# Veason-silverbullet/DIGAT

Hardware: AMD Instinct MI355X
Metric: MIND dev impressions scored/sec (AUC match not run) (higher is better)
Workload: dtype f32; 1 GPU; MIND-small default: --graph_encoder=DIGAT neighbors=3 hops=2 (N=10, U=67), d=400, graph_depth=3, fp32 dev inference; projection=auto -> fp16x3, N=10, U=67, d=400, graph_depth=3, news_num=65238, parallelism=dp1 (row shards, no data-path collective), ranks_in_process_group=1

## Files before the change

digat_amd/_lib.py:

```python
from __future__ import annotations

import ctypes as C
import os
from typing import Optional

import torch

_HERE = os.path.dirname(os.path.abspath(__file__))
LIB_PATH = os.environ.get("DIGAT_HIP_LIB") or os.path.join(_HERE, "lib", "libdigat_hip.so")
DIGAT_MAX_DEPTH = 16
DIGAT_MAX_NODES = 128
GEMM_BF16X6, GEMM_F16X3 = 0, 1
GEMM_F16F8C = 2
PARAMS_GEMM_F16X3 = 64
PARAMS_BD_TILED = 128
PARAMS_PQ_FP8 = 256
PARAMS_SIDE_STREAM_OFF, PARAMS_SIDE_STREAM_ON = 512, 1024
PARAMS_NO_LIVE_ROWS = 2048
PARAMS_PROJ_F16F8C = 4096

_f = C.c_void_p


class LayerParams(C.Structure):
    _fields_ = [(k, _f) for k in ("W", "bW", "F1", "F2", "F3", "b3", "a", "wsplit", "f3_wsplit")]


class MsaParams(C.Structure):
    _fields_ = ([(k, C.c_int32) for k in ("word_embedding_dim", "head_num", "head_dim", "attention_dim")]
                + [(k, C.c_void_p) for k in ("word_embedding", "W_Q", "b_Q", "W_K", "W_V", "b_V", "A1", "b1", "a2",
                                             "qkv_wsplit", "a1_wsplit")])


class CnnParams(C.Structure):
    _fields_ = ([(k, C.c_int32) for k in ("word_embedding_dim", "kernel_num", "taps", "attention_dim")]
                + [(k, C.c_void_p) for k in ("word_embedding", "W", "b", "A1", "b1", "a2", "w_split", "a1_wsplit")])


class SplitJob(C.Structure):
    _fields_ = [("w0", C.c_void_p), ("w1", C.c_void_p), ("w2", C.c_void_p), ("rows", C.c_int32), ("cols", C.c_int32), ("layout", C.c_int32),
                ("reserved", C.c_int32), ("image", C.c_void_p)]


class GatherJob(C.Structure):
    _fields_ = [("src", C.c_void_p), ("dst", C.c_void_p), ("row_bytes", C.c_int64), ("rows", C.c_int64),
                ("idx", C.c_void_p), ("idx2", C.c_void_p), ("inner", C.c_int64)]


class Params(C.Structure):
    _fields_ = ([("d", C.c_int32), ("depth", C.c_int32), ("category_num", C.c_int32), ("flags", C.c_int32)]
                + [(k, _f) for k in ("topic_node_embedding", "cand_K", "cand_Q", "cand_bQ",
                                     "news_graph_W", "news_graph_b", "user_news_K", "user_news_Q",
# ... 107 lines not shown
    "digat_xattn_pairwise_bwd_workspace": (C.c_size_t, [C.c_int] * 3),
    "digat_xattn_pairwise_bwd": (C.c_int, [_f] * 11 + [C.c_float] + [_f] * 4 + [C.c_int] * 4 + [_f, C.c_size_t, _f]),
    "digat_sum_nodes": (C.c_int, [_f, _f, C.c_int, C.c_int, C.c_int, _f]),
    "digat_xattn_train_save_bytes": (C.c_size_t, [C.c_int] * 3),
    "digat_xattn_train_workspace_bytes": (C.c_size_t, [C.c_int] * 3),
    "digat_xattn_fwd_train": (C.c_int, [_f] * 11 + [C.c_float, C.c_uint32, C.c_float, C.c_uint32] + [C.c_int] * 3 + [_f, C.c_size_t, _f, C.c_size_t, _f, C.c_int,
                                        _f]),
    "digat_xattn_bwd": (C.c_int, [_f] * 10 + [C.c_float, C.c_float, _f, C.c_size_t] + [_f] * 9 + [C.c_int] * 3 + [_f, C.c_size_t, _f, C.c_int, _f]),
    "digat_opt_chunk": (C.c_int, []),
    "digat_clip_adam_step": (C.c_int, [_f, _f, _f, C.c_int, _f] + [C.c_float] * 5 + [C.c_int, _f]),
    "digat_row_logits_bwd": (C.c_int, [_f] * 5 + [C.c_int, C.c_int, _f]),
    "digat_click_loss": (C.c_int, [_f, C.c_int, C.c_int, _f, _f, _f]),
    "digat_split_job_bytes": (C.c_size_t, [C.c_int] * 4),
    "digat_split_jobs": (C.c_int, [C.POINTER(SplitJob), C.c_int, _f]),
    "digat_news_ctx_train_save_bytes": (C.c_size_t, [C.c_int] * 3),
    "digat_news_ctx_train_workspace_bytes": (C.c_size_t, [C.c_int] * 3),
    "digat_news_ctx_fwd_train": (C.c_int, [_f] * 8 + [C.c_float, C.c_uint32] + [C.c_int] * 3 + [_f, C.c_size_t, _f, C.c_size_t, _f, _f]),
    "digat_news_ctx_bwd": (C.c_int, [_f] * 6 + [C.c_float, _f, C.c_size_t] + [_f] * 6 + [C.c_int] * 4 + [_f, C.c_size_t, _f]),
    "digat_user_ctx_train_save_bytes": (C.c_size_t, [C.c_int] * 5),
    "digat_user_ctx_train_workspace_bytes": (C.c_size_t, [C.c_int] * 5),
    "digat_user_ctx_fwd_train": (C.c_int, [_f] * 13 + [C.c_float, C.c_uint32] + [C.c_int] * 5 + [_f, C.c_size_t, _f, C.c_size_t, _f, _f, _f]),
    "digat_user_ctx_bwd": (C.c_int, [_f] * 10 + [C.c_float, _f, C.c_size_t] + [_f] * 10 + [C.c_int] * 6 + [_f, C.c_size_t, _f, _f]),
    "digat_profile_start": (C.c_int, [C.c_int]),
    "digat_profile_stop": (C.c_int, [C.POINTER(C.c_double), C.POINTER(C.c_double), C.POINTER(C.c_int)]),
    "digat_profile_set_kinds": (C.c_int, [C.c_uint]),
    "digat_profile_gemm_bytes": (C.c_int, [C.POINTER(C.c_double)]),
    "digat_profile_marker": (C.c_int, [C.c_int, _f]),
    "digat_encoder_shared_workspace_bytes": (C.c_size_t, [C.c_int] * 6),
    "digat_encoder_fwd_shared": (C.c_int, [C.POINTER(Params)] + [_f] * 10 + [C.c_int] * 3 + [_f, C.c_size_t, _f]),
    "digat_user_row_runs": (C.c_int, [_f] * 4 + [C.c_int] * 5 + [_f] * 4 + [C.c_size_t, _f]),
    "digat_profile_xattn_parts": (C.c_int, [C.POINTER(C.c_double), C.POINTER(C.c_double), C.POINTER(C.c_int)]),
    "digat_split_ctx_fused_bytes": (C.c_size_t, [C.c_int]),
    "digat_split_ctx_fused_weights": (C.c_int, [_f, C.c_int, _f, _f]),
}
KERNEL_KINDS = ("proj", "linear", "xattn", "pool", "topic", "glue", "agg")
XATTN_PARTS = ("twin", "l0", "news", "other")
EXPORTED = tuple(_SIGNATURES)
ABI_VERSION = 4


def lib() -> C.CDLL:
    global _lib
    if _lib is None:
        if not os.path.exists(LIB_PATH):
            raise DigatHipError(
                f"{LIB_PATH} is missing: the HIP extension has not been built "
                "(run `python -m digat_amd.build` or __graft_entry__.build()). There is no CPU fallback.")
        handle = C.CDLL(LIB_PATH)
        handle.digat_version.restype, handle.digat_version.argtypes = C.c_int, []
        got = handle.digat_version()
        if got != ABI_VERSION:
            raise DigatHipError(f"{LIB_PATH} reports ABI version {got}, this loader's signature table is for version {ABI_VERSION}: "
                                "rebuild it from this tree (python -m digat_amd.build)")
        for name, (res, args) in _SIGNATURES.items():
            fn = getattr(handle, name)
            fn.restype, fn.argtypes = res, args
        _lib = handle
    return _lib


EXT_PATH = os.path.join(_HERE, "lib", "digat_torch_ext.so")
USE_TORCH_EXT = os.environ.get("DIGAT_TORCH_EXT", "1") != "0"
_ext = None


def ext():
# ... 97 lines not shown
```

digat_amd/csrc/digat_kernels.hip:

```cpp
#include <hip/hip_runtime.h>
#include <stdint.h>
#include <string.h>
#include <stdlib.h>
#include <atomic>
#include <initializer_list>
#include <mutex>
#include <unordered_map>
#include <utility>

#include "../../include/digat_hip.h"

typedef float v4f __attribute__((ext_vector_type(4)));

#define DIGAT_CHECK_LAUNCH()                                   \
    do {                                                       \
        if (hipGetLastError() != hipSuccess) return DIGAT_ERR_LAUNCH; \
    } while (0)

static inline size_t align_up(size_t v, size_t a) { return (v + a - 1) / a * a; }
struct Arena {
    char* base; size_t cap, used; bool ok;
    Arena() : base(nullptr), cap(SIZE_MAX), used(0), ok(true) {}
    Arena(void* p, size_t n) : base((char*)p), cap(n), used(0), ok(p != nullptr) {}
    template <class T> T* take(size_t count) {
// ... 102 lines not shown
}
__device__ __forceinline__ void wait_vmcnt(int n) {
    switch (n) {
        case 0: asm volatile("s_waitcnt vmcnt(0)" ::: "memory"); break;
        case 1: asm volatile("s_waitcnt vmcnt(1)" ::: "memory"); break;
        case 2: asm volatile("s_waitcnt vmcnt(2)" ::: "memory"); break;
        case 3: asm volatile("s_waitcnt vmcnt(3)" ::: "memory"); break;
        case 4: asm volatile("s_waitcnt vmcnt(4)" ::: "memory"); break;
        case 5: asm volatile("s_waitcnt vmcnt(5)" ::: "memory"); break;
        case 6: asm volatile("s_waitcnt vmcnt(6)" ::: "memory"); break;
        default: asm volatile("s_waitcnt vmcnt(4)" ::: "memory"); break;
    }
}

#ifndef DIGAT_TWIN_R
#define DIGAT_TWIN_R 2
#endif
__device__ __forceinline__ float leaky02_uniform(float e) {
    const float t = 0.2f * e;
    float r;
    asm("v_max_f32 %0, %1, %2" : "=v"(r) : "s"(e), "v"(t));
    return r;
}
__device__ __forceinline__ unsigned hash32(unsigned x) {
    x ^= x >> 16; x *= 0x7feb352dU; x ^= x >> 15; x *= 0x846ca68bU; x ^= x >> 16;
    return x;
}
__host__ __device__ __forceinline__ unsigned drop_threshold(float p) { return (unsigned)(p * 4294967296.0); }
__device__ __forceinline__ bool drop_keep(unsigned seed, long e, unsigned thr) {
    return hash32((unsigned)e * 0x9E3779B9U + hash32(seed + (unsigned)(e >> 32))) >= thr;
}
constexpr int TWIN_R = DIGAT_TWIN_R;
#include "digat_gemm.inc"
#include "digat_xattn.inc"
#include "digat_context.inc"
#include "digat_ctxfused.inc"
#include "digat_glue.inc"

extern "C" {

int digat_version(void) { return DIGAT_ABI_VERSION; }

const char* digat_error_string(int code) {
    switch (code) {
        case DIGAT_OK: return "ok";
        case DIGAT_ERR_ARG: return "bad argument (null pointer or negative size)";
        case DIGAT_ERR_SHAPE: return "unsupported shape (d % 4 != 0, graph larger than DIGAT_MAX_NODES, depth too large)";
        case DIGAT_ERR_WORKSPACE: return "workspace too small";
        case DIGAT_ERR_LAUNCH: return "HIP kernel launch failed";
        default: return "unknown error";
    }
}

int digat_linear_f32(const float* x, int64_t ldx, const float* w, const float* b, float* y, int64_t ldy,
                     int M, int N, int K, void* stream) {
    if (!x || !w || !y || M < 0 || N <= 0 || K <= 0) return DIGAT_ERR_ARG;
    if (K % 4 || ldx % 4) return DIGAT_ERR_SHAPE;
    return launch_gemm(gemm_plain(x, ldx, w, b, y, ldy, M, N, K, 0), (hipStream_t)stream);
}

struct XattnWs { float *h, *P, *Q, *r, *alpha; };
static XattnWs xattn_carve(Arena& a, int B, int n, int d) {
    const size_t nd = (size_t)B * n * d;
    XattnWs w{};
    w.h = a.take<float>(3 * nd);
    if (w.h) { w.P = w.h + nd; w.Q = w.P + nd; }
    w.r = a.take<float>((size_t)B * d);
    w.alpha = a.take<float>((size_t)B * n * n);
    return w;
}
size_t digat_xattn_workspace_bytes(int B, int n, int d) { Arena a; xattn_carve(a, B, n, d); return a.used; }

int digat_xattn_pairwise_fwd(const float* Pr, const float* Q, const float* h, const float* X,
                             const float* a, const uint8_t* A, float* out, float* alpha,
                             int B, int n, int d, void* stream) {
    if (!Pr || !Q || !h || !X || !a || !A || !out || !alpha) return DIGAT_ERR_ARG;
    return launch_xattn_pairwise(Pr, Q, h, X, a, A, out, alpha, B, n, d, (hipStream_t)stream);
}

struct TwinLists { const unsigned* word; const int* list; const int* count; };

struct XattnOpts {
    const void* wsplit = nullptr;
    const int* rowidx = nullptr; const int* nrows_dev = nullptr; const uint8_t* live = nullptr;
    int sparse_mode = DIGAT_XATTN_DENSE; const int* sparse_flag = nullptr;
    int pq_x3 = 0, pq_mode = 0, centre_limit = 0, gemm_format = 0, prof_part = 0;
    unsigned* range_flag = nullptr; const TwinLists* tw = nullptr;
};

static int xattn_core(const float* X, const uint8_t* A, const float* r_given,
                      const float* W, const float* bW, const float* F1, const float* F2, const float* a,
// ... 485 lines not shown
    const bool xu0_grouped = Xg0 != nullptr;
    const int d = p->d, C = p->category_num, L = p->depth, U = H + C, C1 = C + 1;
    const int fmt = (p->flags & DIGAT_PARAMS_GEMM_F16X3) ? 1 : 0;
    unsigned* const rflag = fmt ? (unsigned*)p->range_flag : nullptr;
    const int lfmt = (p->flags & DIGAT_PARAMS_PROJ_F16F8C) ? DIGAT_GEMM_F16F8C : fmt;
    const int bd_disp = (p->flags & DIGAT_PARAMS_BD_TILED) ? (1 << 30) : 1;
    float *T = w.fc.T, *T2 = w.fc.T2, *glob = w.fc.glob;
    const int* bucket_idx = nullptr;
    const int* nbuckets_dev = nullptr;
    const int* hist_last = nullptr;
    int rc;
    auto from_c_n = [&](int next_layer, hipStream_t sq) -> int {
        GemmArgs g = gemm_plain(next_layer == 0 ? c_n_src : c_n, d, p->user_news_fold_W, p->user_news_fold_b, w.kq_t, d, B, d, d, 0);
        g.w[1] = p->userAtt_fold_W; g.bias[1] = p->userAtt_fold_b; g.y[1] = w.kq_u;
        g.nsegs = 2;
        if (next_layer < L) {
            g.w[2] = p->user[next_layer].F3; g.bias[2] = p->user[next_layer].b3; g.y[2] = w.r_user[next_layer & 1];
            g.nsegs = 3;
        }
        g.wsplit = (const unsigned short*)p->ctx_wsplit[next_layer]; g.format = fmt; g.range_flag = rflag;
        g.m_dispatch = bd_disp;
        return launch_gemm(g, sq);
    };
    auto user_ctx_tail = [&](const float* Xu_cur, const float* addend, hipStream_t sq, const int* xgroup = nullptr,
                             const uint8_t* live = nullptr, const float* kq_topic = nullptr, const float* kq_user = nullptr) -> int {
        if (!kq_topic) { kq_topic = w.kq_t; kq_user = w.kq_u; }
        if (p->featureAffine_fsplit && fmt == 1 && ctxfused_ok(H, C1, d)) {
            const CtxFusedArgs fa{Xu_cur, (long)U * d, xgroup, live, U, live ? hist_last : nullptr, kq_topic, kq_user, cat_idx, cat_mask, addend, c_u,
                                  (const uint4*)p->featureAffine_fsplit, p->featureAffine_b, rflag, B, H, C1, d, sqrtf((float)d)};
            return launch_user_ctx_fused(fa, sq);
        }
        int e = launch_topic(Xu_cur, (long)U * d, kq_topic, cat_idx, T, B, H, C1, d, sq, xgroup, live, U, live ? hist_last : nullptr);
        if (e) return e;
        GemmArgs g = gemm_plain(T, d, p->featureAffine_W, p->featureAffine_b, T2, d, B * C1, d, d, 0);
        g.epi = EPI_RELU_RES; g.e0 = T; g.lde0 = d;
        g.wsplit = (const unsigned short*)p->featureAffine_wsplit;
        g.format = fmt; g.range_flag = rflag;
        if (bucket_idx && gemm_takes_row_list(g)) { g.rowidx = bucket_idx; g.nrows_dev = nbuckets_dev; }
        e = launch_gemm(g, sq);
        if (e) return e;
        return launch_pool(T2, (long)C1 * d, kq_user, cat_mask, addend, c_u, B, C1, d, sq);
    };
    auto news_ctx = [&](const float* Xn_cur, hipStream_t sq, bool first) -> int {
        const long ldx = (long)N * d;
        float* kq = w.kq_t;
        GemmArgs gq = gemm_plain(Xn_cur, ldx, p->cand_fold_W, p->cand_fold_b, kq, d, B, d, d, 0);
        gq.wsplit = (const unsigned short*)p->cand_fold_wsplit; gq.format = fmt; gq.range_flag = rflag;
        gq.m_dispatch = bd_disp;
        int e = launch_gemm(gq, sq);
        if (e) return e;
        e = launch_pool(Xn_cur, ldx, kq, Mn, nullptr, glob, B, N, d, sq);
        if (e) return e;
        GemmArgs g = gemm_plain(Xn_cur, ldx, p->news_graph_W, p->news_graph_b, c_n, d, B, d, 2 * d, 0);
        g.k0 = d; g.a1 = glob; g.lda1 = d;
        g.epi = EPI_GATE; g.e0 = Xn_cur; g.lde0 = ldx; g.e1 = glob; g.lde1 = d; g.e2 = first ? c_n_src : c_n; g.lde2 = d;
        g.wsplit = (const unsigned short*)p->gate_wsplit; g.format = fmt; g.range_flag = rflag;
        g.m_dispatch = 1;
        return launch_gemm(g, sq);
    };

    const bool want_live = L > 0 && !(p->flags & DIGAT_PARAMS_NO_LIVE_ROWS);
    int sparse_mode = p->flags & 3;
    if (sparse_mode == 3 || (sparse_mode == DIGAT_XATTN_AUTO && L == 0)) sparse_mode = DIGAT_XATTN_DENSE;
    const int* sparse_flag = nullptr;
    const int pq_x3 = (p->flags & DIGAT_PROJ_PQ_X3) ? 1 : 0;
    const int pq_mode = ((p->flags & DIGAT_PQ_BF16) ? 1 : 0) | ((p->flags & DIGAT_PQ_X1) ? 2 : 0) | ((p->flags & DIGAT_PQ_FP8) ? 4 : 0);
    const bool want_scan = want_live || sparse_mode == DIGAT_XATTN_AUTO;
    const int* rowidx = nullptr;
    const int* nrows_dev = nullptr;
    uint8_t* live_flags = nullptr;
    const int *pend_rowidx = nullptr, *pend_nrows = nullptr, *pend_bidx = nullptr, *pend_nb = nullptr, *pend_hlast = nullptr;

// ... 655 lines not shown
```

digat_amd/graphEncoders.py:

```python
from __future__ import annotations

import contextlib
import math
import threading

import torch
import torch.nn as nn

from . import _lib
from .layers import ScaledDotProductAttention

_TLS = threading.local()


class GraphEncoder(nn.Module):
    def __init__(self, config, news_embedding_dim: int):
        super().__init__()
        self.news_graph_size = config.news_graph_size
        self.user_graph_size = config.max_history_num + config.category_num
        self.max_history_num = config.max_history_num
        self.category_num = config.category_num + 1
        self.news_embedding_dim = news_embedding_dim
        self.graph_depth = config.graph_depth
        self.dropout_rate = float(config.dropout_rate)
# ... 15 lines not shown
class DIGAT(GraphEncoder):
    def __init__(self, config, news_embedding_dim: int):
        super().__init__(config, news_embedding_dim)
        d, L = self.news_embedding_dim, self.graph_depth
        if d % 4 != 0:
            raise ValueError("digat_amd needs news_embedding_dim % 4 == 0 (float4 rows)")
        if L > _lib.DIGAT_MAX_DEPTH or max(self.news_graph_size, self.user_graph_size) > _lib.DIGAT_MAX_NODES:
            raise ValueError("graph_depth <= %d and graph sizes <= %d are supported"
                             % (_lib.DIGAT_MAX_DEPTH, _lib.DIGAT_MAX_NODES))
        self.candidate_attention = ScaledDotProductAttention(d, d, d)
        self.news_graph_W = nn.Linear(d * 2, d, bias=True)
        self.user_news_K = nn.Linear(d, d, bias=False)
        self.user_news_Q = nn.Linear(d, d, bias=True)
        self.featureAffine = nn.Linear(d, d, bias=True)
        self.userAttention = ScaledDotProductAttention(d, d, d)
        for g in ("news", "user"):
            setattr(self, f"{g}_graph_attention_W", nn.ModuleList([nn.Linear(d, d, bias=True) for _ in range(L)]))
            setattr(self, f"{g}_graph_attention_ffn1", nn.ModuleList([nn.Linear(d, d, bias=False) for _ in range(L)]))
            setattr(self, f"{g}_graph_attention_ffn2", nn.ModuleList([nn.Linear(d, d, bias=False) for _ in range(L)]))
            setattr(self, f"{g}_graph_attention_ffn3", nn.ModuleList([nn.Linear(d, d, bias=True) for _ in range(L)]))
            setattr(self, f"{g}_graph_attention_a", nn.ModuleList([nn.Linear(d, 1, bias=False) for _ in range(L)]))
        self._param_block = None
        self.projection_mode = "auto"
        self._resolved_pm = None
        self._range_flag = None
        self.range_fallback = False
        self.corpus_activation_max = None
        self.pass_rows = 4096
        self.user_xattn_mode = "auto"
        self.news_xattn_mode = "auto"
        self.corpus_xattn_hint = {}
        self.side_stream = "auto"
        self.live_rows = True
        self.fused_user_context = False

    def initialize(self):
        super().initialize()
        relu_gain = nn.init.calculate_gain('relu')
        leaky_gain = nn.init.calculate_gain('leaky_relu', 0.2)
        for g in ("news", "user"):
            for i in range(self.graph_depth):
                nn.init.xavier_uniform_(getattr(self, f"{g}_graph_attention_W")[i].weight)
                nn.init.zeros_(getattr(self, f"{g}_graph_attention_W")[i].bias)
                nn.init.xavier_uniform_(getattr(self, f"{g}_graph_attention_a")[i].weight, gain=leaky_gain)
                for f in ("ffn1", "ffn2", "ffn3"):
                    nn.init.xavier_uniform_(getattr(self, f"{g}_graph_attention_{f}")[i].weight, gain=relu_gain)
                nn.init.zeros_(getattr(self, f"{g}_graph_attention_ffn3")[i].bias)
        self.candidate_attention.initialize()
        nn.init.xavier_uniform_(self.news_graph_W.weight)
        nn.init.zeros_(self.news_graph_W.bias)
        nn.init.xavier_uniform_(self.user_news_K.weight)
        nn.init.xavier_uniform_(self.user_news_Q.weight)
        nn.init.zeros_(self.user_news_Q.bias)
        nn.init.xavier_uniform_(self.featureAffine.weight, gain=relu_gain)
        nn.init.zeros_(self.featureAffine.bias)
        self.userAttention.initialize()

    @contextlib.contextmanager
    def launch_options(self, side_stream=None, live_rows=None, shared_users=None):
        table = _TLS.__dict__.setdefault("opts", {})
        prev = table.get(id(self))
        cur = dict(prev or {})
        if side_stream is not None:
            if side_stream not in ("auto", "on", "off"):
                raise ValueError("side_stream must be 'auto', 'on' or 'off'")
            cur["side_stream"] = side_stream
        if live_rows is not None:
            cur["live_rows"] = bool(live_rows)
        if shared_users is not None:
            cur["detect_shared_users"] = bool(shared_users)
        table[id(self)] = cur
        try:
            yield self
        finally:
            if prev is None:
                table.pop(id(self), None)
            else:
                table[id(self)] = prev

    def _launch_option(self, name):
        return _TLS.__dict__.get("opts", {}).get(id(self), {}).get(name, getattr(self, name))

    def resolved_xattn_mode(self, g: str) -> str:
        mode = getattr(self, f"{g}_xattn_mode", "auto")
        return self.corpus_xattn_hint.get(g, "auto") if mode == "auto" else mode

    def _apply(self, fn, *args, **kwargs):
        self._param_block = None
        return super()._apply(fn, *args, **kwargs)

    def _params(self) -> "_lib.Params":
        pm = self.resolved_projection_mode()
        fmt = self.gemm_format()
        ptrs = tuple(p.data_ptr() for p in self.parameters())
        if self._param_block is not None and self._param_block[0] == ptrs and self._param_block[2] == self._fold_key():
            return self._call_block(self._param_block[1])
        for p in self.parameters():
            if p.device.type != "cuda" or p.dtype != torch.float32 or not p.is_contiguous():
                raise _lib.DigatHipError("DIGAT parameters must be contiguous float32 CUDA tensors "
                                         "(call model.cuda()); there is no CPU path")
        P = _lib.Params()
# ... 90 lines not shown
        return _lib.GEMM_BF16X6

    def _auto_base(self) -> str:
        if self.news_embedding_dim % 80 != 0:
            return "bf16x6"
        ws = [m.weight for g in ("news", "user") for f in ("W", "ffn1", "ffn2") for m in getattr(self, f"{g}_graph_attention_{f}")]
        ws.append(self.featureAffine.weight)
        key = tuple((w.data_ptr(), w._version) for w in ws + [self.topic_node_embedding])
        key += (self.corpus_activation_max, self.range_fallback)
        if self._resolved_pm is None or self._resolved_pm[0] != key:
            amax = self.corpus_activation_max
            ok = amax is not None and not self.range_fallback
            if ok:
                wmax = float(torch.stack([w.detach().abs().max() for w in ws]).max())
                tmax = float(self.topic_node_embedding.detach().abs().max())
                ok = wmax < 32.0 and amax < 256.0 and tmax < 256.0
            self._resolved_pm = (key, "fp16x3" if ok else "bf16x6")
        return self._resolved_pm[1]

    def range_flag(self) -> torch.Tensor:
        dev = self.topic_node_embedding.device
        if self._range_flag is None or self._range_flag.device != dev:
            self._range_flag = torch.zeros(1, dtype=torch.int32, device=dev)
        return self._range_flag

    def range_overflowed(self, reset: bool = True) -> bool:
        if self._range_flag is None:
            return False
        hit = bool(int(self._range_flag.item()))
        if reset and hit:
            self._range_flag.zero_()
        return hit

    def _flags(self) -> int:
        pm = self.projection_mode
        return ({"auto": 0, "dense": 1, "sparse": 2}[self.resolved_xattn_mode("user")]
                | (4 if pm in ("bf16x6-pq3", "pq-bf16", "pq-fp8") else 0)
                | (8 if self.resolved_xattn_mode("news") == "sparse" else 0)
                | (16 if pm in ("pq-bf16", "pq-bf16-x1") else 0)
                | (32 if pm == "pq-bf16-x1" else 0)
                | (256 if pm == "pq-fp8" else 0)
                | (_lib.PARAMS_GEMM_F16X3 if self.gemm_format() == _lib.GEMM_F16X3 else 0)
                | (_lib.PARAMS_PROJ_F16F8C if pm == "fp16-fp8c" else 0)
                | (_lib.PARAMS_BD_TILED if self.pass_rows >= 2048 else 0)
                | {"auto": 0, "off": _lib.PARAMS_SIDE_STREAM_OFF, "on": _lib.PARAMS_SIDE_STREAM_ON}[self._launch_option("side_stream")]
                | (0 if self._launch_option("live_rows") else _lib.PARAMS_NO_LIVE_ROWS))

    def _fold_sources(self):
        ca, ua = self.candidate_attention, self.userAttention
        return ((ca.K.weight, ca.Q.weight, ca.Q.bias), (self.user_news_K.weight, self.user_news_Q.weight,
                                                        self.user_news_Q.bias), (ua.K.weight, ua.Q.weight, ua.Q.bias))

    def _fold_key(self):
        key = (self.training, self.resolved_projection_mode(), self.gemm_format()) + tuple(t._version for trio in self._fold_sources() for t in trio)
        for g in ("news", "user"):
            for f in ("W", "ffn1", "ffn2"):
                key += tuple(m.weight._version for m in getattr(self, f"{g}_graph_attention_{f}"))
        return key + (self.featureAffine.weight._version, bool(self.fused_user_context))

    def _fold_attention(self):
        L = _lib.lib()
        d = self.news_embedding_dim
        dev = self.topic_node_embedding.device
        nbytes = L.digat_fold_workspace_bytes(d)
        ws = _lib.workspace(nbytes, dev, "fold")
        out = []
        for K, Q, b in self._fold_sources():
            Wf = torch.empty((d, d), dtype=torch.float32, device=dev)
            bf = torch.empty((d,), dtype=torch.float32, device=dev)
            _lib.check(L.digat_fold_attention(K.data_ptr(), Q.data_ptr(), b.data_ptr(), Wf.data_ptr(), bf.data_ptr(), d,
                                              ws.data_ptr(), nbytes, _lib.stream_ptr()), "digat_fold_attention")
            out += [Wf, bf]
        return out

    def _eval_only(self, what: str):
        if self.training and self.dropout_rate > 0 and torch.is_grad_enabled():
            raise NotImplementedError(
                f"{what}: the HIP path implements eval-mode semantics (dropout = identity); "
                "call model.eval() / torch.no_grad(), or train through digat_amd.training")
# ... 469 lines not shown
```

include/digat_hip.h:

```cpp
#ifndef DIGAT_HIP_H
#define DIGAT_HIP_H

#include <stddef.h>
#include <stdint.h>

#ifdef __cplusplus
extern "C" {
#endif

#define DIGAT_ABI_VERSION 4
#define DIGAT_MAX_NODES 128
#define DIGAT_MAX_DEPTH 16

enum {
    DIGAT_OK = 0,
    DIGAT_ERR_ARG = 1,
    DIGAT_ERR_SHAPE = 2,
    DIGAT_ERR_WORKSPACE = 3,
    DIGAT_ERR_LAUNCH = 4
};

int digat_version(void);
const char* digat_error_string(int code);

// ... 61 lines not shown
    const float *F2;
    const float *F3, *b3;
    const float *a;
    const void  *wsplit;
    const void  *f3_wsplit;
} digat_layer_params;

typedef struct digat_params {
    int32_t d;
    int32_t depth;
    int32_t category_num;
    int32_t flags;
    const float *topic_node_embedding;
    const float *cand_K, *cand_Q, *cand_bQ;
    const float *news_graph_W, *news_graph_b;
    const float *user_news_K, *user_news_Q, *user_news_bQ;
    const float *featureAffine_W, *featureAffine_b;
    const float *userAtt_K, *userAtt_Q, *userAtt_bQ;
    digat_layer_params news[DIGAT_MAX_DEPTH];
    digat_layer_params user[DIGAT_MAX_DEPTH];
    const float *cand_fold_W, *cand_fold_b;
    const float *user_news_fold_W, *user_news_fold_b;
    const float *userAtt_fold_W, *userAtt_fold_b;
    const void  *featureAffine_wsplit;
    const void  *cand_fold_wsplit, *gate_wsplit;
    const void  *ctx_wsplit[DIGAT_MAX_DEPTH + 1];
    uint32_t    *range_flag;
    const void  *featureAffine_fsplit;
} digat_params;

size_t digat_split_ctx_fused_bytes(int d);
int digat_split_ctx_fused_weights(const float* W, int d, void* image, void* stream);

size_t digat_fold_workspace_bytes(int d);
int digat_fold_attention(const float* K, const float* Q, const float* bQ, float* Wf, float* bf, int d,
                         void* workspace, size_t workspace_bytes, void* stream);

size_t digat_encoder_workspace_bytes(int B, int N, int H, int C, int d, int depth);
int digat_encoder_fwd(const digat_params* params,
                      const float* news_graph_embeddings, const uint8_t* news_graph,
                      const uint8_t* news_graph_mask, const float* user_news_embedding,
                      const uint8_t* user_graph, const uint8_t* user_category_mask,
                      const int64_t* user_category_indices, const float* news_graph_context,
                      float* out_news_context, float* out_user_context,
                      int B, int N, int H,
                      void* workspace, size_t workspace_bytes, void* stream);

enum { DIGAT_PARAMS_SIDE_STREAM_OFF = 512, DIGAT_PARAMS_SIDE_STREAM_ON = 1024, DIGAT_PARAMS_NO_LIVE_ROWS = 2048 };
enum { DIGAT_PARAMS_PROJ_F16F8C = 4096 };

size_t digat_encoder_grouped_workspace_bytes(int B, int N, int H, int C, int d, int depth);
int digat_encoder_fwd_grouped(const digat_params* params,
                              const float* news_graph_embeddings, const uint8_t* news_graph,
                              const uint8_t* news_graph_mask, const float* user_news_embedding_groups,
                              const uint8_t* user_graph_groups, const uint8_t* user_category_mask_groups,
                              const int64_t* user_category_indices_groups, const int32_t* row_group,
                              const float* news_graph_context, float* out_news_context, float* out_user_context,
                              int B, int G, int N, int H, void* workspace, size_t workspace_bytes, void* stream);

int digat_news_project0(const digat_params* params, const float* Xn, float* hpq, int M, int N, void* stream);
int digat_user_project0(const digat_params* params, const float* X, float* hpq, int M, void* stream);
int digat_news_context_queries(const digat_params* params, const float* c_n, float* out, int M, void* stream);
int digat_encoder_fwd_grouped_cached(const digat_params* params,
                                     const float* news_graph_embeddings, const uint8_t* news_graph, const uint8_t* news_graph_mask,
                                     const float* user_news_embedding_g, const uint8_t* user_graph_g,
                                     const uint8_t* user_category_mask_g, const int64_t* user_category_indices_g,
                                     const int32_t* row_group, const float* news_graph_context, const float* news_hpq0,
                                     const float* hist_hpq0, const float* topic_hpq0, const float* ctxq0,
                                     const int64_t* news_index, int64_t news_rows,
                                     float* out_news, float* out_user, int B, int G, int N, int H,
                                     void* workspace, size_t workspace_bytes, void* stream);

int digat_row_logits(const float* news_ctx, const float* user_ctx, float* logits, int B, int d, void* stream);

int digat_linear_bwd_input(const float* dy, int64_t lddy, const float* w, float* dx, int64_t lddx,
                           int M, int N, int K, int accumulate, void* stream);
int digat_linear_bwd_input_x3(const float* dy, int64_t lddy, const float* w, float* dx, int64_t lddx,
                              int M, int N, int K, int accumulate, void* wsplit, void* stream);
size_t digat_linear_bwd_weight_workspace(int M, int No, int Ni);
int digat_linear_bwd_weight(const float* dy, int64_t lddy, const float* x, int64_t ldx, float* dW, float* db,
                            int M, int No, int Ni, int accumulate, void* workspace, size_t workspace_bytes,
                            void* stream);
// ... 213 lines not shown
```

Baseline: 38520 impressions/s.

## Add register-resident-activation kernel for user featureAffine GEMM with fused ReLU residual

```diff
diff --git a/digat_amd/_lib.py b/digat_amd/_lib.py
--- a/digat_amd/_lib.py
+++ b/digat_amd/_lib.py
@@ -18,6 +18,7 @@
 PARAMS_SIDE_STREAM_OFF, PARAMS_SIDE_STREAM_ON = 512, 1024
 PARAMS_NO_LIVE_ROWS = 2048
 PARAMS_PROJ_F16F8C = 4096
+PARAMS_NO_RESIDENT_FA = 8192
 
 _f = C.c_void_p
 
@@ -191,6 +192,8 @@
     "digat_profile_xattn_parts": (C.c_int, [C.POINTER(C.c_double), C.POINTER(C.c_double), C.POINTER(C.c_int)]),
     "digat_split_ctx_fused_bytes": (C.c_size_t, [C.c_int]),
     "digat_split_ctx_fused_weights": (C.c_int, [_f, C.c_int, _f, _f]),
+    "digat_feature_affine_rows": (C.c_int, [C.POINTER(Params), _f, _f, _f, _f, C.c_int, _f]),
+    "digat_feature_affine_resident": (C.c_int, [C.POINTER(Params), C.c_int]),
 }
 KERNEL_KINDS = ("proj", "linear", "xattn", "pool", "topic", "glue", "agg")
 XATTN_PARTS = ("twin", "l0", "news", "other")
diff --git a/digat_amd/csrc/digat_faffine.inc b/digat_amd/csrc/digat_faffine.inc
--- /dev/null
+++ b/digat_amd/csrc/digat_faffine.inc
@@ -0,0 +1,193 @@
+constexpr int FA_KT_MAX = 13;
+
+template <int KT>
+__global__ void __launch_bounds__(256, 3) feature_affine_f16x3_kernel(const GemmArgs g) {
+    static_assert(KT >= 3 && KT <= FA_KT_MAX, "80 <= K <= 416");
+    constexpr int NT = 5;
+    constexpr int RING = 3;
+    constexpr int IMG_SLOTS = 2 * 320;
+    constexpr int PIECES = IMG_SLOTS / 64;
+    constexpr int IMG_I = (PIECES + 3) / 4;
+    __shared__ uint4 Bs[RING][IMG_SLOTS];
+
+    const int Mv = g.nrows_dev ? __builtin_amdgcn_readfirstlane(*g.nrows_dev) : g.M;
+    if (g.exec_rows && blockIdx.x == 0 && threadIdx.x == 0) atomicAdd(g.exec_rows, (unsigned long long)Mv);
+    const int m0 = (int)blockIdx.x * 64;
+    if (m0 >= Mv) return;
+
+    const int tid = threadIdx.x, lane = tid & 63, wm = tid >> 6;
+    const int kg = lane >> 4, lr = lane & 15;
+    const int K = g.K;
+    const int strips = g.nseg / 80;
+    const unsigned ldsB = (unsigned)(uintptr_t)(__attribute__((address_space(3))) unsigned char*)&Bs[0][0];
+    const char* const wimg = reinterpret_cast<const char*>(g.wsplit);
+    const unsigned wlane = (unsigned)lane * 16u;
+    const int wu = __builtin_amdgcn_readfirstlane(wm);
+
+    auto issue_b = [&](int step, int buf) {
+        const char* src = wimg + (long)step * (IMG_SLOTS * 16);
+#pragma unroll
+        for (int k = 0; k < IMG_I; ++k) {
+            int q = wu + 4 * k;
+            q = q < PIECES ? q : PIECES - 1;
+            lds_dma16_s(src + q * 1024, wlane, ldsB + (unsigned)((buf * IMG_SLOTS + q * 64) * 16));
+        }
+    };
+    issue_b(0, 0);
+    issue_b(1, 1);
+
+    const int gv = m0 + wm * 16 + lr;
+    const bool rok = gv < Mv;
+    const int gvc = rok ? gv : Mv - 1;
+    const int gm = g.rowidx ? g.rowidx[gvc] : gvc;
+    const unsigned rowoff = (unsigned)gm * (unsigned)g.lda0 * 4u + (unsigned)kg * 16u;
+    const float* const arow = reinterpret_cast<const float*>(reinterpret_cast<const char*>(g.a0) + (size_t)((unsigned)gm * (unsigned)g.lda0 * 4u));
+
+    uint4 ahi[KT], alo[KT];
+    float amax = 0.f;
+#pragma unroll
+    for (int kt = 0; kt < KT; ++kt) {
+        int c0 = kt * 32 + kg * 8, c1 = c0 + 4;
+        if (kt == KT - 1) { c0 = c0 < K ? c0 : kg * 8; c1 = c1 < K ? c1 : kg * 8 + 4; }
+        const float4 v0 = *reinterpret_cast<const float4*>(arow + c0);
+        const float4 v1 = *reinterpret_cast<const float4*>(arow + c1);
+        constexpr float xs = F16_ACT_SCALE;
+        const float raw[8] = {v0.x, v0.y, v0.z, v0.w, v1.x, v1.y, v1.z, v1.w};
+        const float v[8] = {v0.x * xs, v0.y * xs, v0.z * xs, v0.w * xs, v1.x * xs, v1.y * xs, v1.z * xs, v1.w * xs};
+        amax = fmaxf(fmaxf(amax, fabsf(v[0])), fabsf(v[1])); amax = fmaxf(fmaxf(amax, fabsf(v[2])), fabsf(v[3]));
+        amax = fmaxf(fmaxf(amax, fabsf(v[4])), fabsf(v[5])); amax = fmaxf(fmaxf(amax, fabsf(v[6])), fabsf(v[7]));
+        unsigned hi[4], lo[4];
+#pragma unroll
+        for (int e = 0; e < 4; ++e) {
+            hi[e] = pack_half_rtz(v[2 * e], v[2 * e + 1]);
+            const fp16x2 h = __builtin_bit_cast(fp16x2, hi[e]);
+            const _Float16 l0 = (_Float16)__builtin_fmaf(raw[2 * e], xs, -(float)h[0]), l1 = (_Float16)__builtin_fmaf(raw[2 * e + 1], xs, -(float)h[1]);
+            lo[e] = (unsigned)__builtin_bit_cast(unsigned short, l0) | ((unsigned)__builtin_bit_cast(unsigned short, l1) << 16);
+        }
+        ahi[kt] = make_uint4(hi[0], hi[1], hi[2], hi[3]);
+        alo[kt] = make_uint4(lo[0], lo[1], lo[2], lo[3]);
+    }
+    if (g.range_flag && __builtin_amdgcn_ballot_w64(!(amax < 65504.f)) != 0 && lane == 0) atomicOr(g.range_flag, 1u);
+
+    auto mma = [&](const uint4 w, const uint4 a, const v4f c) -> v4f {
+        return __builtin_amdgcn_mfma_f32_16x16x32_f16(__builtin_bit_cast(half8, w), __builtin_bit_cast(half8, a), c, 0, 0, 0);
+    };
+    const char* const bp = reinterpret_cast<const char*>(g.bias[0]);
+    char* const ybase = reinterpret_cast<char*>(g.y[0]);
+    const char* const ebase = reinterpret_cast<const char*>(g.e0);
+    const int lslot = kg * 80 + lr;
+
+    int buf = 0;
+    for (int s = 0; s < strips; ++s) {
+        const bool last = s + 1 == strips;
+        v4f acc[NT];
+#pragma unroll
+        for (int nt = 0; nt < NT; ++nt) acc[nt] = (v4f){0.f, 0.f, 0.f, 0.f};
+#pragma unroll
+        for (int kt = 0; kt < KT; ++kt) {
+            if ((kt == 0 && s > 0) || (kt == KT - 1 && last)) asm volatile("s_waitcnt vmcnt(0)" ::: "memory");
+            else wait_vmcnt_imm<IMG_I>();
+            __builtin_amdgcn_s_barrier();
+            if (kt < KT - 2 || !last) issue_b(s * KT + kt + 2, buf == 0 ? RING - 1 : buf - 1);
+            const uint4* Bi = Bs[buf];
+            uint4 bq[2][2];
+#pragma unroll
+            for (int p = 0; p < 2; ++p) bq[0][p] = Bi[p * 320 + lslot];
+#pragma unroll
+            for (int nt = 0; nt < NT; ++nt) {
+                if (nt + 1 < NT) {
+#pragma unroll
+                    for (int p = 0; p < 2; ++p) bq[(nt + 1) & 1][p] = Bi[p * 320 + lslot + (nt + 1) * 16];
+                }
+                const uint4 whi = bq[nt & 1][0], wlo = bq[nt & 1][1];
+                v4f c = acc[nt];
+                c = mma(whi, alo[kt], c);
+                c = mma(wlo, ahi[kt], c);
+                c = mma(whi, ahi[kt], c);
+                acc[nt] = c;
+            }
+            buf = buf == RING - 1 ? 0 : buf + 1;
+        }
+        unsigned ro = rowoff;
+        asm volatile("" : "+v"(ro));
+        const int sb = s * 320;
+        {
+            float4 bv[NT];
+#pragma unroll
+            for (int nt = 0; nt < NT; ++nt) bv[nt] = *reinterpret_cast<const float4*>(bp + sb + (size_t)((unsigned)kg * 16u) + nt * 64);
+#pragma unroll
+            for (int nt = 0; nt < NT; ++nt) {
+                constexpr float u = 1.f / (F16_WEIGHT_SCALE * F16_ACT_SCALE);
+                const float4 v = f4_add(make_float4(acc[nt][0] * u, acc[nt][1] * u, acc[nt][2] * u, acc[nt][3] * u), bv[nt]);
+                acc[nt] = (v4f){v.x, v.y, v.z, v.w};
+            }
+        }
+        asm volatile("" ::: "memory");
+#pragma unroll
+        for (int n0 = 0; n0 < NT; n0 += 3) {
+            float4 ev[3];
+#pragma unroll
+            for (int i = 0; i < 3; ++i)
+                if (n0 + i < NT) ev[i] = *reinterpret_cast<const float4*>(ebase + sb + (size_t)ro + (n0 + i) * 64);
+            if (rok) {
+#pragma unroll
+                for (int i = 0; i < 3; ++i)
+                    if (n0 + i < NT) {
+                        const v4f a = acc[n0 + i];
+                        *reinterpret_cast<float4*>(ybase + sb + (size_t)ro + (n0 + i) * 64) =
+                            make_float4(fmaxf(a[0], 0.f) + ev[i].x, fmaxf(a[1], 0.f) + ev[i].y, fmaxf(a[2], 0.f) + ev[i].z, fmaxf(a[3], 0.f) + ev[i].w);
+                    }
+            }
+            asm volatile("" ::: "memory");
+        }
+    }
+}
+
+static bool feature_affine_ok(const GemmArgs& g) {
+    if (g.format != DIGAT_GEMM_F16X3 || !g.wsplit || g.nsegs != 1 || g.nseg % 80 != 0 || g.K != g.nseg || g.K > 32 * FA_KT_MAX || g.epi != EPI_RELU_RES ||
+        !g.e0 || !g.bias[0] || g.a1 || g.radd || g.gather_only || g.x1_segs || g.x3_segs || g.bf16_segs || g.fp8_segs || g.dmask || g.lda0 % 4 != 0 || g.lde0 != g.lda0 || g.ldy != g.lda0 ||
+        (unsigned long long)g.M * (unsigned long long)g.lda0 * 4ull >= (1ull << 32) ||
+        (((uintptr_t)g.a0 | (uintptr_t)g.e0 | (uintptr_t)g.y[0] | (uintptr_t)g.bias[0]) & 15) != 0)
+        return false;
+    const GemmPlan p = gemm_plan(g);
+    if (p.status != DIGAT_OK || wsplit_format_of(g.wsplit) == DIGAT_GEMM_BF16X6) return false;
+    return p.kernel == GEMM_STRIP_1_F16 || p.kernel == GEMM_STRIP_1_F16_64 || p.kernel == GEMM_STRIP_3_F16_FULL || p.kernel == GEMM_STRIP_3_F16_64;
+}
+
+static int launch_feature_affine(GemmArgs g, hipStream_t st) {
+    if (g.M <= 0) return DIGAT_OK;
+    const int kind = DIGAT_KERNEL_LINEAR;
+    const bool listed = g.rowidx != nullptr;
+    if (listed && g_prof.enabled) {
+        g.exec_rows = g_prof.rows_dev + kind;
+        g_prof.flops_per_row[kind] = 2.0 * (double)g.nseg * g.K; g_prof.rows_nominal[kind] += g.M;
+        g_prof.bytes_per_row[kind] = gemm_row_bytes(g);
+    }
+    ProfScope prof(kind, listed ? 0.0 : 2.0 * g.M * (double)g.nseg * g.K, st, listed ? 0.0 : (double)g.M * gemm_row_bytes(g));
+    const dim3 grid((unsigned)((g.M + 63) / 64));
+    switch ((g.K + 31) >> 5) {
+#define DIGAT_FA_LAUNCH(KT) case KT: hipLaunchKernelGGL(feature_affine_f16x3_kernel<KT>, grid, dim3(256), 0, st, g); break;
+        DIGAT_FA_LAUNCH(3) DIGAT_FA_LAUNCH(5) DIGAT_FA_LAUNCH(8) DIGAT_FA_LAUNCH(10) DIGAT_FA_LAUNCH(13)
+#undef DIGAT_FA_LAUNCH
+        default: return DIGAT_ERR_ARG;
+    }
+    DIGAT_CHECK_LAUNCH();
+    return DIGAT_OK;
+}
+
+static GemmArgs feature_affine_args(const digat_params* p, const float* T, float* y, int M, const int* rows, const int* nrows_dev) {
+    const int d = p->d, fmt = (p->flags & DIGAT_PARAMS_GEMM_F16X3) ? 1 : 0;
+    GemmArgs g = gemm_plain(T, d, p->featureAffine_W, p->featureAffine_b, y, d, M, d, d, 0);
+    g.epi = EPI_RELU_RES; g.e0 = T; g.lde0 = d;
+    g.wsplit = (const unsigned short*)p->featureAffine_wsplit;
+    g.format = fmt; g.range_flag = fmt ? (unsigned*)p->range_flag : nullptr;
+    if (rows && gemm_takes_row_list(g)) { g.rowidx = rows; g.nrows_dev = nrows_dev; }
+    return g;
+}
+static bool feature_affine_resident(const digat_params* p, const GemmArgs& g) {
+    return !(p->flags & DIGAT_PARAMS_NO_RESIDENT_FA) && feature_affine_ok(g);
+}
+static int launch_user_feature_affine(const digat_params* p, const float* T, float* y, int M, const int* rows, const int* nrows_dev, hipStream_t st) {
+    const GemmArgs g = feature_affine_args(p, T, y, M, rows, nrows_dev);
+    return feature_affine_resident(p, g) ? launch_feature_affine(g, st) : launch_gemm(g, st);
+}
diff --git a/digat_amd/csrc/digat_kernels.hip b/digat_amd/csrc/digat_kernels.hip
--- a/digat_amd/csrc/digat_kernels.hip
+++ b/digat_amd/csrc/digat_kernels.hip
@@ -158,6 +158,7 @@
 }
 constexpr int TWIN_R = DIGAT_TWIN_R;
 #include "digat_gemm.inc"
+#include "digat_faffine.inc"
 #include "digat_xattn.inc"
 #include "digat_context.inc"
 #include "digat_ctxfused.inc"
@@ -183,6 +184,18 @@
     if (!x || !w || !y || M < 0 || N <= 0 || K <= 0) return DIGAT_ERR_ARG;
     if (K % 4 || ldx % 4) return DIGAT_ERR_SHAPE;
     return launch_gemm(gemm_plain(x, ldx, w, b, y, ldy, M, N, K, 0), (hipStream_t)stream);
+}
+
+int digat_feature_affine_rows(const digat_params* p, const float* T, float* y, const int* rows, const int* nrows_dev, int M, void* stream) {
+    if (!p || !T || !y || M < 0 || !p->featureAffine_W || (rows == nullptr) != (nrows_dev == nullptr)) return DIGAT_ERR_ARG;
+    if (p->d <= 0 || p->d % 4) return DIGAT_ERR_SHAPE;
+    return launch_user_feature_affine(p, T, y, M, rows, nrows_dev, (hipStream_t)stream);
+}
+
+int digat_feature_affine_resident(const digat_params* p, int M) {
+    if (!p || M <= 0 || p->d <= 0 || p->d % 4) return 0;
+    const float* const T = reinterpret_cast<const float*>((uintptr_t)256);
+    return feature_affine_resident(p, feature_affine_args(p, T, const_cast<float*>(T), M, nullptr, nullptr)) ? 1 : 0;
 }
 
 struct XattnWs { float *h, *P, *Q, *r, *alpha; };
@@ -734,12 +747,7 @@
         }
         int e = launch_topic(Xu_cur, (long)U * d, kq_topic, cat_idx, T, B, H, C1, d, sq, xgroup, live, U, live ? hist_last : nullptr);
         if (e) return e;
-        GemmArgs g = gemm_plain(T, d, p->featureAffine_W, p->featureAffine_b, T2, d, B * C1, d, d, 0);
-        g.epi = EPI_RELU_RES; g.e0 = T; g.lde0 = d;
-        g.wsplit = (const unsigned short*)p->featureAffine_wsplit;
-        g.format = fmt; g.range_flag = rflag;
-        if (bucket_idx && gemm_takes_row_list(g)) { g.rowidx = bucket_idx; g.nrows_dev = nbuckets_dev; }
-        e = launch_gemm(g, sq);
+        e = launch_user_feature_affine(p, T, T2, B * C1, bucket_idx, nbuckets_dev, sq);
         if (e) return e;
         return launch_pool(T2, (long)C1 * d, kq_user, cat_mask, addend, c_u, B, C1, d, sq);
     };
diff --git a/digat_amd/graphEncoders.py b/digat_amd/graphEncoders.py
--- a/digat_amd/graphEncoders.py
+++ b/digat_amd/graphEncoders.py
@@ -71,6 +71,7 @@
         self.corpus_xattn_hint = {}
         self.side_stream = "auto"
         self.live_rows = True
+        self.resident_feature_affine = True
         self.fused_user_context = False
 
     def initialize(self):
@@ -96,7 +97,7 @@
         self.userAttention.initialize()
 
     @contextlib.contextmanager
-    def launch_options(self, side_stream=None, live_rows=None, shared_users=None):
+    def launch_options(self, side_stream=None, live_rows=None, shared_users=None, resident_feature_affine=None):
         table = _TLS.__dict__.setdefault("opts", {})
         prev = table.get(id(self))
         cur = dict(prev or {})
@@ -106,6 +107,8 @@
             cur["side_stream"] = side_stream
         if live_rows is not None:
             cur["live_rows"] = bool(live_rows)
+        if resident_feature_affine is not None:
+            cur["resident_feature_affine"] = bool(resident_feature_affine)
         if shared_users is not None:
             cur["detect_shared_users"] = bool(shared_users)
         table[id(self)] = cur
@@ -262,6 +265,20 @@
             self._range_flag.zero_()
         return hit
 
+    def feature_affine_rows(self, T, rows=None, nrows=None, out=None):
+        T = _lib.f32(T)
+        dev = _lib.require_device(T)
+        out = torch.empty_like(T) if out is None else out
+        if (rows is None) != (nrows is None) or any(t is not None and t.dtype != torch.int32 for t in (rows, nrows)):
+            raise ValueError("rows and nrows: int32 device tensors, both or neither")
+        if T.shape[0]:
+            _lib.check(_lib.lib().digat_feature_affine_rows(self._params(), T.data_ptr(), out.data_ptr(), _lib.ptr(rows), _lib.ptr(nrows),
+                                                            T.shape[0], _lib.stream_ptr()), "digat_feature_affine_rows")
+        return out
+
+    def feature_affine_resident(self, rows: int) -> bool:
+        return bool(_lib.lib().digat_feature_affine_resident(self._params(), int(rows)))
+
     def _flags(self) -> int:
         pm = self.projection_mode
         return ({"auto": 0, "dense": 1, "sparse": 2}[self.resolved_xattn_mode("user")]
@@ -274,7 +291,8 @@
                 | (_lib.PARAMS_PROJ_F16F8C if pm == "fp16-fp8c" else 0)
                 | (_lib.PARAMS_BD_TILED if self.pass_rows >= 2048 else 0)
                 | {"auto": 0, "off": _lib.PARAMS_SIDE_STREAM_OFF, "on": _lib.PARAMS_SIDE_STREAM_ON}[self._launch_option("side_stream")]
-                | (0 if self._launch_option("live_rows") else _lib.PARAMS_NO_LIVE_ROWS))
+                | (0 if self._launch_option("live_rows") else _lib.PARAMS_NO_LIVE_ROWS)
+                | (0 if self._launch_option("resident_feature_affine") else _lib.PARAMS_NO_RESIDENT_FA))
 
     def _fold_sources(self):
         ca, ua = self.candidate_attention, self.userAttention
diff --git a/include/digat_hip.h b/include/digat_hip.h
--- a/include/digat_hip.h
+++ b/include/digat_hip.h
@@ -117,6 +117,9 @@
 size_t digat_split_ctx_fused_bytes(int d);
 int digat_split_ctx_fused_weights(const float* W, int d, void* image, void* stream);
 
+int digat_feature_affine_rows(const digat_params* params, const float* T, float* y, const int* rows, const int* nrows_dev, int M, void* stream);
+int digat_feature_affine_resident(const digat_params* params, int M);
+
 size_t digat_fold_workspace_bytes(int d);
 int digat_fold_attention(const float* K, const float* Q, const float* bQ, float* Wf, float* bf, int d,
                          void* workspace, size_t workspace_bytes, void* stream);
@@ -133,6 +136,7 @@
 
 enum { DIGAT_PARAMS_SIDE_STREAM_OFF = 512, DIGAT_PARAMS_SIDE_STREAM_ON = 1024, DIGAT_PARAMS_NO_LIVE_ROWS = 2048 };
 enum { DIGAT_PARAMS_PROJ_F16F8C = 4096 };
+enum { DIGAT_PARAMS_NO_RESIDENT_FA = 8192 };
 
 size_t digat_encoder_grouped_workspace_bytes(int B, int N, int H, int C, int d, int depth);
 int digat_encoder_fwd_grouped(const digat_params* params,
```

Result: faster. 38940 impressions/s, median of 6 (+1.1%).
